# facebookresearch/generative-recommenders

Measured on NVIDIA H100. Metric: user-seqs/sec HSTU-large L=8192 d=256 bf16 fwd+bwd, higher is better.
Workload: dtype bf16

## Files before the change

### generative_recommenders_b200/_lib.py

```python
import ctypes as C
import os
from typing import Optional

import torch

_HERE = os.path.dirname(os.path.abspath(__file__))
LIB_PATH = os.environ.get("HSTU_B200_LIB") or os.path.join(_HERE, "lib", "libhstu_b200.so")

ABI_VERSION = 1
F32, BF16, F16, E4M3 = 0, 1, 2, 3
IMPL_AUTO, IMPL_GENERIC, IMPL_UMMA = 0, 1, 2

_DTYPES = {torch.float32: F32, torch.bfloat16: BF16, torch.float16: F16, torch.float8_e4m3fn: E4M3}


class AttnParams(C.Structure):
    _fields_ = [
        ("abi_version", C.c_int32), ("dtype", C.c_int32), ("impl", C.c_int32), ("batch", C.c_int32),
        ("heads", C.c_int32), ("dqk", C.c_int32), ("dv", C.c_int32), ("max_seq_len", C.c_int32),
        ("total_rows", C.c_int64), ("alpha", C.c_float), ("max_attn_len", C.c_int32),
        ("min_full_attn_seq_len", C.c_int32), ("contextual_seq_len", C.c_int32), ("delta_q_len", C.c_int32),
        ("offsets_are_i64", C.c_int32), ("num_targets_are_i64", C.c_int32),
        ("seq_offsets", C.c_void_p), ("num_targets", C.c_void_p), ("q", C.c_void_p), ("k", C.c_void_p),
        ("v", C.c_void_p), ("out", C.c_void_p),
# ... 28 lines not shown
    ]


_lib: Optional[C.CDLL] = None

_i32, _i64, _f32, _u64, _vp = C.c_int32, C.c_int64, C.c_float, C.c_uint64, C.c_void_p

_PROTOS = {
    "hstu_last_error": (C.c_char_p, []),
    "hstu_abi_version": (C.c_int, []),
    "hstu_attn_workspace_bytes": (C.c_size_t, [C.POINTER(AttnParams), C.c_int]),
    "hstu_attn_fwd": (C.c_int, [C.POINTER(AttnParams), _vp]),
    "hstu_attn_bwd": (C.c_int, [C.POINTER(AttnParams), _vp]),
    "hstu_attn_fwd_fp8": (C.c_int, [C.POINTER(AttnParams), C.POINTER(Descales), _vp]),
    "hstu_attn_select_impl": (C.c_int, [C.POINTER(AttnParams), C.c_int]),
    "hstu_mask_valid": (C.c_int, [_i32] * 7),
    "hstu_kv_range_for_q_rows": (C.c_int, [_i32] * 7 + [C.POINTER(_i32)] * 2),
    "hstu_q_range_for_kv_rows": (C.c_int, [_i32] * 7 + [C.POINTER(_i32)] * 3),
    "hstu_layer_norm_fwd": (C.c_int, [_vp, _vp, _vp, _vp, _vp, _vp, _i64, _i32, _i64, _i64, _f32, _i32, _i32, _vp]),
    "hstu_layer_norm_bwd": (C.c_int, [_vp] * 10 + [_i64, _i32, _i64, _i64, _i64, _i32, _i32, _vp]),
    "hstu_norm_bwd_partial_rows": (_i32, []),
    "hstu_rms_norm_fwd": (C.c_int, [_vp, _vp, _vp, _vp, _i64, _i32, _f32, _i32, _vp]),
    "hstu_rms_norm_bwd": (C.c_int, [_vp] * 7 + [_i64, _i32, _i32, _vp]),
    "hstu_norm_mul_dropout_fwd": (C.c_int, [_vp] * 7 + [_i64, _i32, _i32, _i64, _i64, _f32, _f32, _u64, _i32, _i32, _i32, _i32, _vp]),
    "hstu_norm_mul_dropout_bwd": (C.c_int, [_vp] * 12 + [_i64, _i32, _i32, _i64, _i64, _i64, _i64, _f32, _u64, _i32, _i32, _i32, _i32, _vp]),
    "hstu_silu_fwd": (C.c_int, [_vp, _vp, _i64, _i32, _i64, _i64, _i32, _vp]),
    "hstu_silu_bwd": (C.c_int, [_vp, _vp, _vp, _i64, _i32, _i64, _i64, _i64, _i32, _vp]),
    "hstu_jagged_concat": (C.c_int, [_vp] * 5 + [_i32] * 8 + [_vp]),
    "hstu_jagged_split": (C.c_int, [_vp] * 5 + [_i32] * 8 + [_vp]),
    "hstu_position_embeddings_fwd": (C.c_int, [_vp] * 10 + [_i64, _i32, _i32, _i32, _i32, _i32, _f32, _i32, _i32, _i32, _i32, _i32, _i32, _vp]),
# ... 117 lines not shown
```

### generative_recommenders_b200/csrc/api.cu

```cuda
#include <stdarg.h>
#include <string.h>

#include "common.cuh"
#include "internal.h"

namespace hstu {

static thread_local char g_err[512] = "";

void set_error(const char* fmt, ...) {
  va_list ap;
  va_start(ap, fmt);
  vsnprintf(g_err, sizeof(g_err), fmt, ap);
  va_end(ap);
}

static int validate_attn(const hstu_attn_params* p, bool bwd) {
  HSTU_CHECK_ARG(p != nullptr, "params is NULL");
  HSTU_CHECK_ARG(p->abi_version == HSTU_B200_ABI_VERSION, "ABI version mismatch: caller %d, library %d", p->abi_version,
                 HSTU_B200_ABI_VERSION);
  HSTU_CHECK_ARG(p->dtype == HSTU_F32 || p->dtype == HSTU_BF16 || p->dtype == HSTU_F16 || p->dtype == HSTU_E4M3, "bad dtype %d",
                 p->dtype);
  HSTU_CHECK_ARG(p->max_seq_len > 0, "max_seq_len must be larger than 0");
  HSTU_CHECK_ARG(p->batch >= 0 && p->heads > 0, "bad batch/heads");
// ... 45 lines not shown
    set_error("deterministic backward with a relative bias is not supported: the dpos_w / dts_w gradients are added "
              "with atomics");
    return HSTU_ERR_UNSUPPORTED;
  }
  const bool can = wgmma_supported(*p, bwd);
  if (p->impl == HSTU_IMPL_GENERIC) return HSTU_IMPL_GENERIC;
  if (p->impl == HSTU_IMPL_UMMA) {
    if (!can) {
      set_error("wgmma path does not support this problem (dtype=%d dqk=%d dv=%d delta=%d bias=%d)", p->dtype, p->dqk,
                p->dv, p->delta_q_len, p->pos_w != nullptr || p->ts_w != nullptr);
      return HSTU_ERR_UNSUPPORTED;
    }
    return HSTU_IMPL_UMMA;
  }
  return can ? HSTU_IMPL_UMMA : HSTU_IMPL_GENERIC;
}

static int validate_descales(const hstu_attn_descales* d) {
  if (d == nullptr) return 0;
  const float* ptr[3] = {d->q, d->k, d->v};
  const int64_t bs[3] = {d->q_batch_stride, d->k_batch_stride, d->v_batch_stride};
  const int64_t hs[3] = {d->q_head_stride, d->k_head_stride, d->v_head_stride};
  for (int i = 0; i < 3; ++i) {
    const char name = "qkv"[i];
    HSTU_CHECK_ARG(bs[i] >= 0 && hs[i] >= 0, "%c descale: negative stride (batch %lld, head %lld)", name, (long long)bs[i],
                   (long long)hs[i]);
    HSTU_CHECK_ARG((reinterpret_cast<uintptr_t>(ptr[i]) & 3) == 0, "%c descale: %p is not a float pointer", name, (const void*)ptr[i]);
  }
  return 0;
}
// ... 69 lines not shown
  if (int e = validate_attn(p, false)) return e;
  HSTU_CHECK_ARG(p->dtype == HSTU_E4M3, "hstu_attn_fwd_fp8: q, k, v must be HSTU_E4M3 (got dtype %d)", p->dtype);
  if (int e = validate_descales(descales)) return e;
  const int impl = select_impl(p, false);
  if (impl < 0) return impl;
  if (p->batch == 0 || p->total_rows == 0) return 0;
  if (int e = bind_device(p->q)) return e;
  if (int e = check_descale_devices(descales)) return e;
  if (!is_sm90()) {
    set_error("hstu_attn_fwd_fp8: the fp8 kernels need an sm_90 device");
    return HSTU_ERR_UNSUPPORTED;
  }
  hstu_attn_descales none;
  memset(&none, 0, sizeof(none));
  return attn_wgmma_fwd_e4m3(*p, descales ? *descales : none, (cudaStream_t)stream);
}

int hstu_mask_valid(int32_t len, int32_t num_targets, int32_t max_attn_len, int32_t min_full_attn_seq_len,
                    int32_t contextual_seq_len, int32_t i, int32_t j) {
  SeqMask m = make_seq_mask(len, num_targets, max_attn_len, min_full_attn_seq_len, contextual_seq_len);
  return mask_valid(m, i, j) ? 1 : 0;
}

int hstu_kv_range_for_q_rows(int32_t len, int32_t num_targets, int32_t max_attn_len, int32_t min_full_attn_seq_len,
                             int32_t contextual_seq_len, int32_t m0, int32_t m1, int32_t* lo, int32_t* hi) {
  HSTU_CHECK_ARG(lo && hi && m0 >= 0 && m1 > m0 && m1 <= len, "bad row range");
  SeqMask m = make_seq_mask(len, num_targets, max_attn_len, min_full_attn_seq_len, contextual_seq_len);
  int l, h;
  kv_range_for_q_rows(m, m0, m1, &l, &h);
  *lo = l;
// ... 202 lines not shown
```

### generative_recommenders_b200/csrc/attn_fp16_operands.cu

```cuda
#include <cuda_fp16.h>
#include <cuda_fp8.h>
#include <string.h>

#include "attn_fp16_operands.cuh"
#include "common.cuh"
#include "internal.h"

namespace hstu {

constexpr int kPreRows = 256, kPreThreads = 256, kPreD = 32;

struct PreOperand {
  const void* src;
  long long row_stride, head_stride;
  __half* dst;
};

struct PreParams {
  PreOperand op[kAmaxSlots];
  int nops;
  const void* seq_offsets;
  int offsets_i64, max_seq_len, heads;
  int d;
  float alpha;
  uint32_t* amax;
};

__device__ __forceinline__ float bf16_bits_to_float(uint32_t b) { return __uint_as_float(b << 16); }

__global__ void __launch_bounds__(kPreThreads) fp16_operands_amax_kernel(const __grid_constant__ PreParams p) {
  const int b = blockIdx.z, h = blockIdx.y;
  const long long row0 = load_index(p.seq_offsets, p.offsets_i64, b);
  const int len = min((int)(load_index(p.seq_offsets, p.offsets_i64, b + 1) - row0), p.max_seq_len);
  const int r0 = blockIdx.x * kPreRows;
  if (r0 >= len) return;
// ... 11 lines not shown
#pragma unroll
      for (int i = 0; i < 4; ++i) {
        m = max(m, (w[i] & 0x7fffu) << 16);
        m = max(m, (w[i] >> 16 & 0x7fffu) << 16);
      }
    }
#pragma unroll
    for (int s = 16; s > 0; s >>= 1) m = max(m, __shfl_xor_sync(0xffffffffu, m, s));
    if (lane == 0) red[o][warp] = m;
  }
  __syncthreads();
  if (threadIdx.x < p.nops) {
    uint32_t m = 0u;
#pragma unroll
    for (int w = 0; w < kPreThreads / 32; ++w) m = max(m, red[threadIdx.x][w]);
    if (m) atomicMax(p.amax + ((long long)b * p.heads + h) * kAmaxSlots + threadIdx.x, m);
  }
}

template <bool E4M3>
__global__ void __launch_bounds__(kPreThreads) fp16_operands_convert_kernel(const __grid_constant__ PreParams p) {
  const int b = blockIdx.z, h = blockIdx.y;
  const long long row0 = load_index(p.seq_offsets, p.offsets_i64, b);
  const int len = min((int)(load_index(p.seq_offsets, p.offsets_i64, b + 1) - row0), p.max_seq_len);
  const int r0 = blockIdx.x * kPreRows;
  if (r0 >= len) return;
  const int rows = min(kPreRows, len - r0);
  const int d = E4M3 ? p.d : kPreD, cpr = d / 8;
  int exps[kAmaxSlots] = {0, 0, 0, 0};
  if constexpr (!E4M3) {
    const OperandExps ex = operand_exps(p.amax + ((long long)b * p.heads + h) * kAmaxSlots, p.alpha, kPreD);
    exps[0] = ex.q, exps[1] = ex.k, exps[2] = ex.v, exps[3] = ex.o;
  }
  for (int o = 0; o < p.nops; ++o) {
    const PreOperand& op = p.op[o];
    const int e = exps[o];
    for (int c = threadIdx.x; c < rows * cpr; c += kPreThreads) {
      const int r = c / cpr, part = c % cpr;
      const long long row = row0 + r0 + r;
      uint32_t y[4];
      if constexpr (E4M3) {
        const uint2 x = *reinterpret_cast<const uint2*>(reinterpret_cast<const uint8_t*>(op.src) + row * op.row_stride +
                                                        (long long)h * op.head_stride + part * 8);
        const uint32_t w[2] = {x.x, x.y};
#pragma unroll
        for (int i = 0; i < 4; ++i) {
          const __half2_raw v = __nv_cvt_fp8x2_to_halfraw2((__nv_fp8x2_storage_t)(w[i >> 1] >> (16 * (i & 1))), __NV_E4M3);
          y[i] = (uint32_t)v.x | ((uint32_t)v.y << 16);
        }
      } else {
        const uint4 x = *reinterpret_cast<const uint4*>(reinterpret_cast<const uint16_t*>(op.src) + row * op.row_stride +
                                                        (long long)h * op.head_stride + part * 8);
        const uint32_t w[4] = {x.x, x.y, x.z, x.w};
#pragma unroll
        for (int i = 0; i < 4; ++i) {
          const __half2 v = __floats2half2_rn(scalbnf(bf16_bits_to_float(w[i] & 0xffffu), e), scalbnf(bf16_bits_to_float(w[i] >> 16), e));
          y[i] = *reinterpret_cast<const uint32_t*>(&v);
        }
      }
      *reinterpret_cast<uint4*>(op.dst + (row * p.heads + h) * d + part * 8) = make_uint4(y[0], y[1], y[2], y[3]);
    }
  }
}

static size_t align256(size_t n) { return (n + 255) / 256 * 256; }

size_t fp16_operands_workspace_bytes(const hstu_attn_params& p, bool bwd) {
  const size_t amax = align256((size_t)p.batch * p.heads * kAmaxSlots * sizeof(uint32_t));
  const size_t copy = align256((size_t)p.total_rows * p.heads * kPreD * sizeof(__half));
  return amax + (bwd ? 4 : 3) * copy;
}

int fp16_operands_prepass(const hstu_attn_params& p, bool bwd, Fp16Operands* out, cudaStream_t st) {
  const size_t need = fp16_operands_workspace_bytes(p, bwd);
  if (p.workspace == nullptr || p.workspace_bytes < need) {
    set_error("hstu_attn_%s: workspace of %zu bytes required (got %zu)", bwd ? "bwd" : "fwd", need, p.workspace_bytes);
    return HSTU_ERR_WORKSPACE;
  }
  uint8_t* ws = reinterpret_cast<uint8_t*>(p.workspace);
  const size_t amax_bytes = (size_t)p.batch * p.heads * kAmaxSlots * sizeof(uint32_t);
  const size_t copy = align256((size_t)p.total_rows * p.heads * kPreD * sizeof(__half));
  PreParams pp;
  memset(&pp, 0, sizeof(pp));
  pp.amax = reinterpret_cast<uint32_t*>(ws);
  const void* src[kAmaxSlots] = {p.q, p.k, p.v, p.dout};
  const long long rs[kAmaxSlots] = {p.q_row_stride, p.k_row_stride, p.v_row_stride, p.do_row_stride};
  const long long hs[kAmaxSlots] = {p.q_head_stride, p.k_head_stride, p.v_head_stride, p.do_head_stride};
  pp.nops = bwd ? 4 : 3;
  for (int o = 0; o < pp.nops; ++o) {
    pp.op[o].src = src[o];
    pp.op[o].row_stride = rs[o];
    pp.op[o].head_stride = hs[o];
    pp.op[o].dst = reinterpret_cast<__half*>(ws + align256(amax_bytes) + o * copy);
    out->copy[o] = pp.op[o].dst;
  }
  out->amax = pp.amax;
  pp.seq_offsets = p.seq_offsets;
  pp.offsets_i64 = p.offsets_are_i64;
  pp.max_seq_len = p.max_seq_len;
  pp.heads = p.heads;
  pp.alpha = p.alpha;
  HSTU_CUDA_OK(cudaMemsetAsync(pp.amax, 0, amax_bytes, st));
  if (p.batch == 0 || p.max_seq_len <= 0) return 0;
  const dim3 grid((p.max_seq_len + kPreRows - 1) / kPreRows, p.heads, p.batch);
  fp16_operands_amax_kernel<<<grid, kPreThreads, 0, st>>>(pp);
  HSTU_CUDA_OK(cudaGetLastError());
  fp16_operands_convert_kernel<false><<<grid, kPreThreads, 0, st>>>(pp);
  HSTU_CUDA_OK(cudaGetLastError());
  return 0;
}

size_t e4m3_v_copy_bytes(const hstu_attn_params& p) { return align256((size_t)p.total_rows * p.heads * p.dv * sizeof(__half)); }

int e4m3_v_prepass(const hstu_attn_params& p, const void** v16, cudaStream_t st) {
  const size_t need = e4m3_v_copy_bytes(p);
  if (p.workspace == nullptr || p.workspace_bytes < need) {
    set_error("hstu_attn_fwd_fp8: workspace of %zu bytes required (got %zu)", need, p.workspace_bytes);
    return HSTU_ERR_WORKSPACE;
  }
  PreParams pp;
  memset(&pp, 0, sizeof(pp));
  pp.nops = 1;
  pp.op[0].src = p.v;
  pp.op[0].row_stride = p.v_row_stride;
// ... 17 lines not shown
```

### generative_recommenders_b200/csrc/attn_wgmma_bwd.cu

```cuda
#include "attn_wgmma_bwd.cuh"

namespace hstu {

template <int D, bool BF16>
__global__ void __launch_bounds__(kAttnThreads, 1) attn_bwd_wgmma_kernel(const __grid_constant__ BwdParams p) {
  bwd_key_tile<D, D, BF16, true>(p);
}

template <int D, bool BF16>
__global__ void __launch_bounds__(kAttnThreads, split_min_blocks(D)) attn_bwd_dkdv_wgmma_kernel(const __grid_constant__ BwdParams p) {
  bwd_key_tile<D, D, BF16, false>(p);
}

template <int D, bool BF16>
__global__ void __launch_bounds__(kAttnThreads, split_min_blocks(D)) attn_bwd_dq_wgmma_kernel(const __grid_constant__ BwdParams p) {
  bwd_dq_body<D, D, BF16>(p);
}

template <bool BF16>
__global__ void dq_convert_kernel(const float* __restrict__ acc, uint16_t* __restrict__ dq, long long rows, int heads, int D,
                                  long long row_stride, long long head_stride, float scale) {
  const long long nvec = rows * heads * (D / 8);
  for (long long idx = (long long)blockIdx.x * blockDim.x + threadIdx.x; idx < nvec; idx += (long long)gridDim.x * blockDim.x) {
    const int v = (int)(idx % (D / 8));
// ... 88 lines not shown
      return launch_bwd_wgmma<32, false, true>(p, st, &f16);
    }
    case 64:
      if (split) return bf ? launch_bwd_wgmma<64, true, true>(p, st) : launch_bwd_wgmma<64, false, true>(p, st);
      return bf ? launch_bwd_wgmma<64, true, false>(p, st) : launch_bwd_wgmma<64, false, false>(p, st);
    case 128:
      if (split) return bf ? launch_bwd_wgmma<128, true, true>(p, st) : launch_bwd_wgmma<128, false, true>(p, st);
      return bf ? launch_bwd_wgmma<128, true, false>(p, st) : launch_bwd_wgmma<128, false, false>(p, st);
    case 256:
      return bf ? launch_bwd_wgmma<256, true, true>(p, st) : launch_bwd_wgmma<256, false, true>(p, st);
  }
  set_error("wgmma backward: unsupported head dim %d", p.dqk);
  return HSTU_ERR_UNSUPPORTED;
}

}
```

### generative_recommenders_b200/csrc/internal.h

```cpp
#pragma once
#include <cuda_runtime.h>
#include <stddef.h>

#include "../../include/hstu_b200.h"

namespace hstu {
void set_error(const char* fmt, ...);

int attn_generic_fwd(const hstu_attn_params& p, cudaStream_t st);
int attn_generic_bwd(const hstu_attn_params& p, cudaStream_t st);

bool wgmma_supported(const hstu_attn_params& p, bool bwd);
size_t wgmma_workspace_bytes(const hstu_attn_params& p, bool bwd);
int attn_wgmma_fwd(const hstu_attn_params& p, cudaStream_t st);
int attn_wgmma_bwd(const hstu_attn_params& p, cudaStream_t st);
int attn_wgmma_fwd_mixed(const hstu_attn_params& p, cudaStream_t st);
int attn_wgmma_bwd_mixed(const hstu_attn_params& p, cudaStream_t st);
bool aligned_view(const void* ptr, long long row_stride, long long head_stride);
bool wgmma_fwd_supported(const hstu_attn_params& p);
size_t wgmma_delta_workspace_bytes(const hstu_attn_params& p);

struct Fp16Operands {
  const unsigned int* amax;
  const void* copy[4];
};
size_t fp16_operands_workspace_bytes(const hstu_attn_params& p, bool bwd);
int fp16_operands_prepass(const hstu_attn_params& p, bool bwd, Fp16Operands* out, cudaStream_t st);
size_t e4m3_v_copy_bytes(const hstu_attn_params& p);
int e4m3_v_prepass(const hstu_attn_params& p, const void** v16, cudaStream_t st);

int e4m3_fwd_check(const hstu_attn_params& p);
int attn_wgmma_fwd_e4m3(const hstu_attn_params& p, const hstu_attn_descales& ds, cudaStream_t st);
int attn_wgmma_fwd_e4m3_mixed(const hstu_attn_params& p, const hstu_attn_descales& ds, const void* v16, cudaStream_t st);
bool is_sm90();

int layer_norm_fwd(const void* x, const void* w, const void* b, void* y, float* mean, float* rstd, long long n, int D,
                   long long xs, long long ys, float eps, int dtype, int swish, bool rms, cudaStream_t st);
int layer_norm_bwd(const void* dy, const void* x, const void* w, const void* b, const float* mean, const float* rstd,
                   void* dx, float* dw, float* db, float* partial, long long n, int D, long long xs, long long dys,
                   long long dxs, int dtype, int swish, bool rms, cudaStream_t st);
int norm_mul_dropout_fwd(const void* attn, const void* u, const void* w, const void* b, void* out, float* mean,
                         float* rstd, long long n, int H, int dv, long long as, long long us, float eps, float p,
// ... 46 lines not shown
```

### generative_recommenders_b200/ops/hstu_attention.py

```python
import ctypes as C
from typing import Optional, Tuple

import torch

from .. import _lib
from ..common import HammerKernel, require_cuda_kernel, switch_to_contiguous_if_needed


def _fill_common(p, max_seq_len, alpha, q, k, v, seq_offsets, num_targets, max_attn_len, contextual_seq_len,
                 min_full_attn_seq_len, impl, delta_q_len=0):
    if seq_offsets.dtype not in (torch.int32, torch.int64):
        raise RuntimeError("seq_offsets must be int32 or int64")
    if num_targets is not None and num_targets.dtype not in (torch.int32, torch.int64):
        raise RuntimeError("num_targets must be int32 or int64")
    p.abi_version = _lib.ABI_VERSION
    p.dtype = _lib.dtype_code(q)
    p.impl = impl
    p.batch = seq_offsets.numel() - 1
    p.heads = q.shape[1]
    p.dqk = q.shape[2]
    p.dv = v.shape[2]
    p.max_seq_len = int(max_seq_len)
    p.total_rows = k.shape[0]
    p.alpha = float(alpha)
# ... 14 lines not shown
def _workspace(p, bwd: bool, device):
    nbytes = _lib.lib().hstu_attn_workspace_bytes(C.byref(p), int(bwd))
    if nbytes == 0:
        p.workspace, p.workspace_bytes = None, 0
        return None
    ws = torch.empty(nbytes + 256, dtype=torch.uint8, device=device)
    base = (ws.data_ptr() + 255) // 256 * 256
    p.workspace, p.workspace_bytes = base, nbytes
    return ws


def _prep(*ts):
    return tuple(switch_to_contiguous_if_needed(t) for t in ts)


def cuda_hstu_attention_fwd(
    max_seq_len: int, alpha: float, q: torch.Tensor, k: torch.Tensor, v: torch.Tensor, seq_offsets: torch.Tensor,
    num_targets: Optional[torch.Tensor] = None, max_attn_len: int = 0, contextual_seq_len: int = 0,
    min_full_attn_seq_len: int = 0, impl: int = _lib.IMPL_AUTO, delta_q_len: int = 0,
    out: Optional[torch.Tensor] = None, bias: Optional[Tuple[torch.Tensor, torch.Tensor, torch.Tensor]] = None,
    descales: Optional[Tuple[Optional[torch.Tensor], Optional[torch.Tensor], Optional[torch.Tensor]]] = None,
) -> torch.Tensor:
    if descales is not None or any(t.dtype == _FP8 for t in (q, k, v)):
        if bias is not None or delta_q_len:
            raise RuntimeError("fp8 attention: the relative bias and delta_q are not supported")
        return cuda_hstu_attention_fwd_fp8(max_seq_len, alpha, q, k, v, seq_offsets, descales, num_targets, max_attn_len,
                                           contextual_seq_len, min_full_attn_seq_len, impl, out)
    dev = _lib.require_cuda(q, k, v, seq_offsets, num_targets)
    q, k, v = _prep(q, k, v)
    seq_offsets = seq_offsets.contiguous()
    if num_targets is not None:
        num_targets = num_targets.contiguous()
    if out is None:
        out = torch.empty((q.shape[0], q.shape[1], v.shape[2]), dtype=v.dtype, device=dev)
    p = _lib.AttnParams()
    _fill_common(p, max_seq_len, alpha, q, k, v, seq_offsets, num_targets, max_attn_len, contextual_seq_len,
                 min_full_attn_seq_len, impl, delta_q_len)
    p.out = out.data_ptr()
    p.o_row_stride, p.o_head_stride = out.stride(0), out.stride(1)
    keep = _fill_bias(p, bias, None)
    ws = _workspace(p, False, dev)
    with torch.cuda.device(dev), _lib.timed("attn_fwd", dev):
        _lib.check(_lib.lib().hstu_attn_fwd(C.byref(p), _lib.stream_ptr(dev)), "hstu_attn_fwd")
    if delta_q_len:
        _lib.note_launch(2 if ws is not None else 1)
    else:
        _lib.note_launch(3 if ws is not None else 1)
    del ws, keep
    return out


_FP8 = torch.float8_e4m3fn


def cuda_hstu_attention_fwd_fp8(
    max_seq_len: int, alpha: float, q: torch.Tensor, k: torch.Tensor, v: torch.Tensor, seq_offsets: torch.Tensor,
    descales: Optional[Tuple[Optional[torch.Tensor], Optional[torch.Tensor], Optional[torch.Tensor]]] = None,
    num_targets: Optional[torch.Tensor] = None, max_attn_len: int = 0, contextual_seq_len: int = 0,
    min_full_attn_seq_len: int = 0, impl: int = _lib.IMPL_AUTO, out: Optional[torch.Tensor] = None,
) -> torch.Tensor:
    if not all(t.dtype == _FP8 for t in (q, k, v)):
        raise RuntimeError(f"fp8 attention: q, k and v must all be torch.float8_e4m3fn (got {q.dtype}, {k.dtype}, {v.dtype}); "
# ... 29 lines not shown
    with torch.cuda.device(dev), _lib.timed("attn_fwd_fp8", dev):
        _lib.check(_lib.lib().hstu_attn_fwd_fp8(C.byref(p), C.byref(ds), _lib.stream_ptr(dev)), "hstu_attn_fwd_fp8")
    _lib.note_launch(2)
    del ws
    return out


def cuda_hstu_attention_bwd(
    max_seq_len: int, alpha: float, dout: torch.Tensor, q: torch.Tensor, k: torch.Tensor, v: torch.Tensor,
    dq: torch.Tensor, dk: torch.Tensor, dv: torch.Tensor, seq_offsets: torch.Tensor,
    num_targets: Optional[torch.Tensor] = None, max_attn_len: int = 0, contextual_seq_len: int = 0,
    min_full_attn_seq_len: int = 0, impl: int = _lib.IMPL_AUTO,
    bias: Optional[Tuple[torch.Tensor, torch.Tensor, torch.Tensor]] = None,
    dbias: Optional[Tuple[torch.Tensor, torch.Tensor]] = None,
    deterministic: Optional[bool] = None,
) -> None:
    if deterministic is None:
        deterministic = torch.are_deterministic_algorithms_enabled()
    dev = _lib.require_cuda(dout, q, k, v, dq, dk, dv, seq_offsets, num_targets)
    q, k, v, dout = _prep(q, k, v, dout)
    for g in (dq, dk, dv):
        if g.stride(-1) != 1:
            raise RuntimeError("dq/dk/dv must have a dense last dimension")
    seq_offsets = seq_offsets.contiguous()
    if num_targets is not None:
        num_targets = num_targets.contiguous()
    p = _lib.AttnParams()
    _fill_common(p, max_seq_len, alpha, q, k, v, seq_offsets, num_targets, max_attn_len, contextual_seq_len,
                 min_full_attn_seq_len, impl)
    p.dout, p.dq, p.dk, p.dv_out = dout.data_ptr(), dq.data_ptr(), dk.data_ptr(), dv.data_ptr()
    p.do_row_stride, p.do_head_stride = dout.stride(0), dout.stride(1)
    p.dq_row_stride, p.dq_head_stride = dq.stride(0), dq.stride(1)
    p.dk_row_stride, p.dk_head_stride = dk.stride(0), dk.stride(1)
    p.dv_row_stride, p.dv_head_stride = dv.stride(0), dv.stride(1)
    p.deterministic = int(bool(deterministic))
    keep = _fill_bias(p, bias, dbias)
    ws = _workspace(p, True, dev)
    with torch.cuda.device(dev), _lib.timed("attn_bwd", dev):
        _lib.check(_lib.lib().hstu_attn_bwd(C.byref(p), _lib.stream_ptr(dev)), "hstu_attn_bwd")
    _lib.note_launch(4 if ws is not None and p.dtype == _lib.BF16 and p.dqk == 32 else 2)
    del ws, keep


def _fill_bias(p, bias, dbias):
    if bias is None:
        return None
    pos_w, ts_w, timestamps = bias
    keep = []
    n, B = int(p.max_seq_len), int(p.batch)
    if pos_w is not None and pos_w.numel() != 2 * n - 1:
        raise RuntimeError(f"relative position bias: pos_w must have 2 * max_seq_len - 1 = {2 * n - 1} entries, got {pos_w.numel()}")
# ... 131 lines not shown
```

### generative_recommenders_b200/ops/hstu_compute.py

```python
from typing import Optional, Tuple

import torch

from .. import _lib
from ..common import HammerKernel, require_cuda_kernel
from .hstu_attention import cuda_hstu_attention_bwd, cuda_hstu_attention_fwd, hstu_mha
from .layer_norm import _partial, cuda_layer_norm_bwd, cuda_layer_norm_fwd, layer_norm


def cuda_silu_fwd(x: torch.Tensor) -> torch.Tensor:
    dev = _lib.require_cuda(x)
    n, c = x.shape
    y = torch.empty((n, c), dtype=x.dtype, device=dev)
    with torch.cuda.device(dev), _lib.timed("silu_fwd", dev):
        _lib.check(_lib.lib().hstu_silu_fwd(x.data_ptr(), y.data_ptr(), n, c, x.stride(0), y.stride(0), _lib.dtype_code(x),
                                            _lib.stream_ptr(dev)), "hstu_silu_fwd")
        _lib.note_launch(1)
    return y


def cuda_silu_bwd(dy: torch.Tensor, x: torch.Tensor, dx: torch.Tensor) -> None:
    dev = x.device
    n, c = x.shape
    dy = dy if dy.stride(-1) == 1 else dy.contiguous()
# ... 130 lines not shown
                                            training, concat_ux, group_norm, num_heads, linear_dim, silu_u,
                                            recompute_y_in_backward)


class _HSTUPreprocessAndAttentionFunction(torch.autograd.Function):
    @staticmethod
    def forward(ctx, x, norm_weight, norm_bias, norm_eps, num_heads, attn_dim, hidden_dim, uvqk_weight, uvqk_bias,
                max_seq_len, seq_offsets, attn_alpha, num_targets, max_attn_len, contextual_seq_len, recompute_uvqk,
                recompute_normed_x, impl):
        x = _row_major(x)
        normed_x, mean, rstd = cuda_layer_norm_fwd(x, norm_weight, norm_bias, norm_eps, False)
        uvqk = torch.addmm(uvqk_bias, normed_x, uvqk_weight)
        H, dqk, dv = num_heads, attn_dim, hidden_dim
        u_pre, v, q, k = torch.split(uvqk, [dv * H, dv * H, dqk * H, dqk * H], dim=1)
        u = cuda_silu_fwd(u_pre)
        out = cuda_hstu_attention_fwd(max_seq_len, attn_alpha, q.view(-1, H, dqk), k.view(-1, H, dqk), v.view(-1, H, dv),
                                      seq_offsets, num_targets, max_attn_len, contextual_seq_len, 0, impl)
        ctx.save_for_backward(x, norm_weight, norm_bias, uvqk_weight, uvqk_bias, mean, rstd, seq_offsets, num_targets,
                              None if recompute_normed_x else normed_x,
                              None if recompute_uvqk else uvqk)
        ctx.cfg = (norm_eps, H, dqk, dv, max_seq_len, attn_alpha, max_attn_len, contextual_seq_len, impl)
        return u, out.view(-1, H * dv)

    @staticmethod
    def backward(ctx, du, dattn):
        (x, norm_weight, norm_bias, uvqk_weight, uvqk_bias, mean, rstd, seq_offsets, num_targets, normed_x,
         uvqk) = ctx.saved_tensors
        norm_eps, H, dqk, dv, max_seq_len, alpha, max_attn_len, contextual_seq_len, impl = ctx.cfg
        if normed_x is None:
            normed_x, _, _ = cuda_layer_norm_fwd(x, norm_weight, norm_bias, norm_eps, False, save_stats=False)
        if uvqk is None:
            uvqk = torch.addmm(uvqk_bias, normed_x, uvqk_weight)
        u_pre, v, q, k = torch.split(uvqk, [dv * H, dv * H, dqk * H, dqk * H], dim=1)
        duvqk = torch.empty_like(uvqk)
        d_u, d_v, d_q, d_k = torch.split(duvqk, [dv * H, dv * H, dqk * H, dqk * H], dim=1)
        dattn = _row_major(dattn)
        cuda_hstu_attention_bwd(max_seq_len, alpha, dattn.view(-1, H, dv), q.view(-1, H, dqk), k.view(-1, H, dqk),
                                v.view(-1, H, dv), d_q.view(-1, H, dqk), d_k.view(-1, H, dqk), d_v.view(-1, H, dv),
                                seq_offsets, num_targets, max_attn_len, contextual_seq_len, 0, impl)
        cuda_silu_bwd(du, u_pre, d_u)
        d_w = torch.mm(normed_x.t(), duvqk)
        d_b = duvqk.sum(dim=0)
        d_normed = torch.mm(duvqk, uvqk_weight.t())
        dx, dnw, dnb = cuda_layer_norm_bwd(d_normed, x, norm_weight, norm_bias, mean, rstd, False)
        return (dx, dnw.to(norm_weight.dtype), dnb.to(norm_bias.dtype), None, None, None, None, d_w, d_b, None, None, None,
                None, None, None, None, None, None)


def hstu_preprocess_and_attention(
    x: torch.Tensor, norm_weight: torch.Tensor, norm_bias: torch.Tensor, norm_eps: float, num_heads: int, attn_dim: int,
    hidden_dim: int, uvqk_weight: torch.Tensor, uvqk_bias: torch.Tensor, max_seq_len: int, seq_offsets: torch.Tensor,
    attn_alpha: float, causal: bool, num_targets: Optional[torch.Tensor], max_attn_len: int, contextual_seq_len: int,
    recompute_uvqk_in_backward: bool, recompute_normed_x_in_backward: bool, sort_by_length: bool, prefill: bool = False,
    kernel: HammerKernel = HammerKernel.CUDA, impl: int = _lib.IMPL_AUTO,
# ... 22 lines not shown
```

### include/hstu_b200.h

```cpp
#ifndef HSTU_B200_H_
#define HSTU_B200_H_

#include <stddef.h>
#include <stdint.h>

#ifdef __cplusplus
extern "C" {
#endif

#define HSTU_B200_ABI_VERSION 1

typedef enum hstu_dtype { HSTU_F32 = 0, HSTU_BF16 = 1, HSTU_F16 = 2, HSTU_E4M3 = 3 } hstu_dtype;

typedef enum hstu_status {
  HSTU_OK = 0,
  HSTU_ERR_INVALID_ARGUMENT = -1,
  HSTU_ERR_UNSUPPORTED = -2,
  HSTU_ERR_CUDA = -3,
  HSTU_ERR_WORKSPACE = -4
} hstu_status;

typedef enum hstu_attn_impl {
  HSTU_IMPL_AUTO = 0,
  HSTU_IMPL_GENERIC = 1,
// ... 40 lines not shown
  const int64_t* timestamps;
  int32_t num_ts_buckets;
  int32_t deterministic;
  float* dpos_w;
  float* dts_w;
  void* workspace;
  size_t workspace_bytes;
} hstu_attn_params;

const char* hstu_last_error(void);
int hstu_abi_version(void);

size_t hstu_attn_workspace_bytes(const hstu_attn_params* p, int is_backward);
int hstu_attn_fwd(const hstu_attn_params* p, void* cuda_stream);
int hstu_attn_bwd(const hstu_attn_params* p, void* cuda_stream);

typedef struct hstu_attn_descales {
  const float* q;
  const float* k;
  const float* v;
  int64_t q_batch_stride, q_head_stride;
  int64_t k_batch_stride, k_head_stride;
  int64_t v_batch_stride, v_head_stride;
} hstu_attn_descales;
int hstu_attn_fwd_fp8(const hstu_attn_params* p, const hstu_attn_descales* descales, void* cuda_stream);
int hstu_attn_select_impl(const hstu_attn_params* p, int is_backward);

int hstu_mask_valid(int32_t len, int32_t num_targets , int32_t max_attn_len,
                    int32_t min_full_attn_seq_len, int32_t contextual_seq_len, int32_t i, int32_t j);
int hstu_kv_range_for_q_rows(int32_t len, int32_t num_targets, int32_t max_attn_len, int32_t min_full_attn_seq_len,
// ... 92 lines not shown
```

Measured before the change: 103.4.

## Keep fp16 attention operands from forward and reuse them in backward

The forward pass can now write its converted fp16 copies of q, k and v, plus their amax scales, into a buffer that is saved on the autograd context. The backward pass then converts only dout and runs the wgmma backward kernel on the kept copies. When uvqk is recomputed, only the u slice is recomputed, skipping the q/k/v part of the addmm. This removes the repeated bf16-to-fp16 prepass and part of the GEMM recompute, at the cost of holding three extra fp16 operand copies in memory between forward and backward. The path is gated to bf16 with dqk == dv == 32 on the wgmma kernels.

```diff
diff --git a/generative_recommenders_b200/_lib.py b/generative_recommenders_b200/_lib.py
--- a/generative_recommenders_b200/_lib.py
+++ b/generative_recommenders_b200/_lib.py
@@ -66,6 +66,10 @@
     "hstu_attn_bwd": (C.c_int, [C.POINTER(AttnParams), _vp]),
     "hstu_attn_fwd_fp8": (C.c_int, [C.POINTER(AttnParams), C.POINTER(Descales), _vp]),
     "hstu_attn_select_impl": (C.c_int, [C.POINTER(AttnParams), C.c_int]),
+    "hstu_attn_fp16_operands_bytes": (C.c_size_t, [C.POINTER(AttnParams)]),
+    "hstu_attn_fwd_keep_fp16_operands": (C.c_int, [C.POINTER(AttnParams), _vp, C.c_size_t, _vp]),
+    "hstu_attn_bwd_fp16_operands_workspace_bytes": (C.c_size_t, [C.POINTER(AttnParams)]),
+    "hstu_attn_bwd_on_fp16_operands": (C.c_int, [C.POINTER(AttnParams), _vp, C.c_size_t, _vp]),
     "hstu_mask_valid": (C.c_int, [_i32] * 7),
     "hstu_kv_range_for_q_rows": (C.c_int, [_i32] * 7 + [C.POINTER(_i32)] * 2),
     "hstu_q_range_for_kv_rows": (C.c_int, [_i32] * 7 + [C.POINTER(_i32)] * 3),
diff --git a/generative_recommenders_b200/csrc/api.cu b/generative_recommenders_b200/csrc/api.cu
--- a/generative_recommenders_b200/csrc/api.cu
+++ b/generative_recommenders_b200/csrc/api.cu
@@ -83,6 +83,10 @@
     return HSTU_IMPL_UMMA;
   }
   return can ? HSTU_IMPL_UMMA : HSTU_IMPL_GENERIC;
+}
+
+static bool runs_on_fp16_operands(const hstu_attn_params* p, bool bwd) {
+  return p->dtype == HSTU_BF16 && p->dqk == 32 && p->dv == 32 && p->delta_q_len == 0 && select_impl(p, bwd) == HSTU_IMPL_UMMA;
 }
 
 static int validate_descales(const hstu_attn_descales* d) {
@@ -182,6 +186,57 @@
   hstu_attn_descales none;
   memset(&none, 0, sizeof(none));
   return attn_wgmma_fwd_e4m3(*p, descales ? *descales : none, (cudaStream_t)stream);
+}
+
+size_t hstu_attn_fp16_operands_bytes(const hstu_attn_params* p) {
+  if (p == nullptr || validate_attn(p, false) != 0) return 0;
+  if (p->batch == 0 || p->total_rows == 0 || !runs_on_fp16_operands(p, false)) return 0;
+  return fp16_operands_workspace_bytes(*p, false);
+}
+
+int hstu_attn_fwd_keep_fp16_operands(const hstu_attn_params* p, void* operands, size_t operands_bytes, void* stream) {
+  if (int e = validate_attn(p, false)) return e;
+  if (p->batch == 0 || p->total_rows == 0) return 0;
+  HSTU_CHECK_ARG(operands != nullptr && (reinterpret_cast<uintptr_t>(operands) & 255) == 0,
+                 "operands must be a 256-byte aligned buffer (got %p)", operands);
+  if (int e = bind_device(p->q)) return e;
+  if (!runs_on_fp16_operands(p, false)) {
+    set_error("hstu_attn_fwd_keep_fp16_operands: only bf16 at dqk == dv == 32 on the wgmma kernels runs on fp16 operands");
+    return HSTU_ERR_UNSUPPORTED;
+  }
+  const size_t need = fp16_operands_workspace_bytes(*p, false);
+  HSTU_CHECK_ARG(operands_bytes >= need, "operands buffer of %zu bytes required (got %zu)", need, operands_bytes);
+  hstu_attn_params c = *p;
+  c.workspace = operands;
+  c.workspace_bytes = need;
+  return attn_wgmma_fwd(c, (cudaStream_t)stream);
+}
+
+size_t hstu_attn_bwd_fp16_operands_workspace_bytes(const hstu_attn_params* p) {
+  if (p == nullptr || p->batch <= 0 || p->heads <= 0 || p->total_rows <= 0) return 0;
+  return fp16_operands_dout_workspace_bytes(*p);
+}
+
+int hstu_attn_bwd_on_fp16_operands(const hstu_attn_params* p, const void* operands, size_t operands_bytes, void* stream) {
+  HSTU_CHECK_ARG(p != nullptr, "params is NULL");
+  HSTU_CHECK_ARG(operands != nullptr && (reinterpret_cast<uintptr_t>(operands) & 255) == 0,
+                 "operands must be a 256-byte aligned buffer (got %p)", operands);
+  hstu_attn_params c = *p;
+  const Fp16Operands kept = fp16_operands_at(c, const_cast<void*>(operands));
+  c.q = kept.copy[0], c.k = kept.copy[1], c.v = kept.copy[2];
+  c.q_row_stride = c.k_row_stride = c.v_row_stride = (int64_t)c.heads * c.dqk;
+  c.q_head_stride = c.k_head_stride = c.v_head_stride = c.dqk;
+  if (int e = validate_attn(&c, true)) return e;
+  if (c.batch == 0 || c.total_rows == 0) return 0;
+  const size_t need = fp16_operands_workspace_bytes(c, false);
+  HSTU_CHECK_ARG(operands_bytes >= need, "operands buffer of %zu bytes required (got %zu): not kept by a forward of these sizes",
+                 need, operands_bytes);
+  if (int e = bind_device(c.dout)) return e;
+  if (!runs_on_fp16_operands(&c, true)) {
+    set_error("hstu_attn_bwd_on_fp16_operands: only bf16 at dqk == dv == 32 on the wgmma kernels runs on fp16 operands");
+    return HSTU_ERR_UNSUPPORTED;
+  }
+  return attn_wgmma_bwd_on_fp16_operands(c, operands, (cudaStream_t)stream);
 }
 
 int hstu_mask_valid(int32_t len, int32_t num_targets, int32_t max_attn_len, int32_t min_full_attn_seq_len,
diff --git a/generative_recommenders_b200/csrc/attn_fp16_operands.cu b/generative_recommenders_b200/csrc/attn_fp16_operands.cu
--- a/generative_recommenders_b200/csrc/attn_fp16_operands.cu
+++ b/generative_recommenders_b200/csrc/attn_fp16_operands.cu
@@ -19,6 +19,7 @@
 struct PreParams {
   PreOperand op[kAmaxSlots];
   int nops;
+  int slot0;
   const void* seq_offsets;
   int offsets_i64, max_seq_len, heads;
   int d;
@@ -60,7 +61,7 @@
     uint32_t m = 0u;
 #pragma unroll
     for (int w = 0; w < kPreThreads / 32; ++w) m = max(m, red[threadIdx.x][w]);
-    if (m) atomicMax(p.amax + ((long long)b * p.heads + h) * kAmaxSlots + threadIdx.x, m);
+    if (m) atomicMax(p.amax + ((long long)b * p.heads + h) * kAmaxSlots + p.slot0 + threadIdx.x, m);
   }
 }
 
@@ -80,7 +81,7 @@
   }
   for (int o = 0; o < p.nops; ++o) {
     const PreOperand& op = p.op[o];
-    const int e = exps[o];
+    const int e = exps[p.slot0 + o];
     for (int c = threadIdx.x; c < rows * cpr; c += kPreThreads) {
       const int r = c / cpr, part = c % cpr;
       const long long row = row0 + r0 + r;
@@ -110,11 +111,36 @@
 }
 
 static size_t align256(size_t n) { return (n + 255) / 256 * 256; }
+static size_t amax_bytes(const hstu_attn_params& p) { return (size_t)p.batch * p.heads * kAmaxSlots * sizeof(uint32_t); }
+static size_t copy_bytes(const hstu_attn_params& p) { return align256((size_t)p.total_rows * p.heads * kPreD * sizeof(__half)); }
 
 size_t fp16_operands_workspace_bytes(const hstu_attn_params& p, bool bwd) {
-  const size_t amax = align256((size_t)p.batch * p.heads * kAmaxSlots * sizeof(uint32_t));
-  const size_t copy = align256((size_t)p.total_rows * p.heads * kPreD * sizeof(__half));
-  return amax + (bwd ? 4 : 3) * copy;
+  return align256(amax_bytes(p)) + (bwd ? 4 : 3) * copy_bytes(p);
+}
+
+size_t fp16_operands_dout_workspace_bytes(const hstu_attn_params& p) { return align256(amax_bytes(p)) + copy_bytes(p); }
+
+Fp16Operands fp16_operands_at(const hstu_attn_params& p, void* buf) {
+  uint8_t* base = reinterpret_cast<uint8_t*>(buf);
+  Fp16Operands f;
+  f.amax = reinterpret_cast<uint32_t*>(base);
+  for (int o = 0; o < kAmaxSlots; ++o) f.copy[o] = base + align256(amax_bytes(p)) + o * copy_bytes(p);
+  return f;
+}
+
+static int launch_prepass(const hstu_attn_params& p, PreParams& pp, cudaStream_t st) {
+  pp.seq_offsets = p.seq_offsets;
+  pp.offsets_i64 = p.offsets_are_i64;
+  pp.max_seq_len = p.max_seq_len;
+  pp.heads = p.heads;
+  pp.alpha = p.alpha;
+  if (p.batch == 0 || p.max_seq_len <= 0) return 0;
+  const dim3 grid((p.max_seq_len + kPreRows - 1) / kPreRows, p.heads, p.batch);
+  fp16_operands_amax_kernel<<<grid, kPreThreads, 0, st>>>(pp);
+  HSTU_CUDA_OK(cudaGetLastError());
+  fp16_operands_convert_kernel<false><<<grid, kPreThreads, 0, st>>>(pp);
+  HSTU_CUDA_OK(cudaGetLastError());
+  return 0;
 }
 
 int fp16_operands_prepass(const hstu_attn_params& p, bool bwd, Fp16Operands* out, cudaStream_t st) {
@@ -123,12 +149,10 @@
     set_error("hstu_attn_%s: workspace of %zu bytes required (got %zu)", bwd ? "bwd" : "fwd", need, p.workspace_bytes);
     return HSTU_ERR_WORKSPACE;
   }
-  uint8_t* ws = reinterpret_cast<uint8_t*>(p.workspace);
-  const size_t amax_bytes = (size_t)p.batch * p.heads * kAmaxSlots * sizeof(uint32_t);
-  const size_t copy = align256((size_t)p.total_rows * p.heads * kPreD * sizeof(__half));
+  *out = fp16_operands_at(p, p.workspace);
   PreParams pp;
   memset(&pp, 0, sizeof(pp));
-  pp.amax = reinterpret_cast<uint32_t*>(ws);
+  pp.amax = const_cast<uint32_t*>(out->amax);
   const void* src[kAmaxSlots] = {p.q, p.k, p.v, p.dout};
   const long long rs[kAmaxSlots] = {p.q_row_stride, p.k_row_stride, p.v_row_stride, p.do_row_stride};
   const long long hs[kAmaxSlots] = {p.q_head_stride, p.k_head_stride, p.v_head_stride, p.do_head_stride};
@@ -137,23 +161,33 @@
     pp.op[o].src = src[o];
     pp.op[o].row_stride = rs[o];
     pp.op[o].head_stride = hs[o];
-    pp.op[o].dst = reinterpret_cast<__half*>(ws + align256(amax_bytes) + o * copy);
-    out->copy[o] = pp.op[o].dst;
-  }
-  out->amax = pp.amax;
-  pp.seq_offsets = p.seq_offsets;
-  pp.offsets_i64 = p.offsets_are_i64;
-  pp.max_seq_len = p.max_seq_len;
-  pp.heads = p.heads;
-  pp.alpha = p.alpha;
-  HSTU_CUDA_OK(cudaMemsetAsync(pp.amax, 0, amax_bytes, st));
-  if (p.batch == 0 || p.max_seq_len <= 0) return 0;
-  const dim3 grid((p.max_seq_len + kPreRows - 1) / kPreRows, p.heads, p.batch);
-  fp16_operands_amax_kernel<<<grid, kPreThreads, 0, st>>>(pp);
-  HSTU_CUDA_OK(cudaGetLastError());
-  fp16_operands_convert_kernel<false><<<grid, kPreThreads, 0, st>>>(pp);
-  HSTU_CUDA_OK(cudaGetLastError());
-  return 0;
+    pp.op[o].dst = reinterpret_cast<__half*>(const_cast<void*>(out->copy[o]));
+  }
+  HSTU_CUDA_OK(cudaMemsetAsync(pp.amax, 0, amax_bytes(p), st));
+  return launch_prepass(p, pp, st);
+}
+
+int fp16_operands_dout_prepass(const hstu_attn_params& p, const void* kept, Fp16Operands* out, cudaStream_t st) {
+  const size_t need = fp16_operands_dout_workspace_bytes(p);
+  if (p.workspace == nullptr || p.workspace_bytes < need) {
+    set_error("hstu_attn_bwd_on_fp16_operands: workspace of %zu bytes required (got %zu)", need, p.workspace_bytes);
+    return HSTU_ERR_WORKSPACE;
+  }
+  const Fp16Operands k = fp16_operands_at(p, const_cast<void*>(kept)), w = fp16_operands_at(p, p.workspace);
+  out->amax = w.amax;
+  for (int o = 0; o < 3; ++o) out->copy[o] = k.copy[o];
+  out->copy[kAmaxDO] = w.copy[0];
+  PreParams pp;
+  memset(&pp, 0, sizeof(pp));
+  pp.amax = const_cast<uint32_t*>(w.amax);
+  pp.nops = 1;
+  pp.slot0 = kAmaxDO;
+  pp.op[0].src = p.dout;
+  pp.op[0].row_stride = p.do_row_stride;
+  pp.op[0].head_stride = p.do_head_stride;
+  pp.op[0].dst = reinterpret_cast<__half*>(const_cast<void*>(w.copy[0]));
+  HSTU_CUDA_OK(cudaMemcpyAsync(pp.amax, k.amax, amax_bytes(p), cudaMemcpyDeviceToDevice, st));
+  return launch_prepass(p, pp, st);
 }
 
 size_t e4m3_v_copy_bytes(const hstu_attn_params& p) { return align256((size_t)p.total_rows * p.heads * p.dv * sizeof(__half)); }
diff --git a/generative_recommenders_b200/csrc/attn_wgmma_bwd.cu b/generative_recommenders_b200/csrc/attn_wgmma_bwd.cu
--- a/generative_recommenders_b200/csrc/attn_wgmma_bwd.cu
+++ b/generative_recommenders_b200/csrc/attn_wgmma_bwd.cu
@@ -126,4 +126,10 @@
   return HSTU_ERR_UNSUPPORTED;
 }
 
+int attn_wgmma_bwd_on_fp16_operands(const hstu_attn_params& p, const void* kept, cudaStream_t st) {
+  Fp16Operands f16;
+  if (int e = fp16_operands_dout_prepass(p, kept, &f16, st)) return e;
+  return launch_bwd_wgmma<32, false, true>(p, st, &f16);
 }
+
+}
diff --git a/generative_recommenders_b200/csrc/internal.h b/generative_recommenders_b200/csrc/internal.h
--- a/generative_recommenders_b200/csrc/internal.h
+++ b/generative_recommenders_b200/csrc/internal.h
@@ -14,6 +14,7 @@
 size_t wgmma_workspace_bytes(const hstu_attn_params& p, bool bwd);
 int attn_wgmma_fwd(const hstu_attn_params& p, cudaStream_t st);
 int attn_wgmma_bwd(const hstu_attn_params& p, cudaStream_t st);
+int attn_wgmma_bwd_on_fp16_operands(const hstu_attn_params& p, const void* kept, cudaStream_t st);
 int attn_wgmma_fwd_mixed(const hstu_attn_params& p, cudaStream_t st);
 int attn_wgmma_bwd_mixed(const hstu_attn_params& p, cudaStream_t st);
 bool aligned_view(const void* ptr, long long row_stride, long long head_stride);
@@ -25,7 +26,10 @@
   const void* copy[4];
 };
 size_t fp16_operands_workspace_bytes(const hstu_attn_params& p, bool bwd);
+Fp16Operands fp16_operands_at(const hstu_attn_params& p, void* buf);
 int fp16_operands_prepass(const hstu_attn_params& p, bool bwd, Fp16Operands* out, cudaStream_t st);
+size_t fp16_operands_dout_workspace_bytes(const hstu_attn_params& p);
+int fp16_operands_dout_prepass(const hstu_attn_params& p, const void* kept, Fp16Operands* out, cudaStream_t st);
 size_t e4m3_v_copy_bytes(const hstu_attn_params& p);
 int e4m3_v_prepass(const hstu_attn_params& p, const void** v16, cudaStream_t st);
 
diff --git a/generative_recommenders_b200/ops/hstu_attention.py b/generative_recommenders_b200/ops/hstu_attention.py
--- a/generative_recommenders_b200/ops/hstu_attention.py
+++ b/generative_recommenders_b200/ops/hstu_attention.py
@@ -52,12 +52,26 @@
     return tuple(switch_to_contiguous_if_needed(t) for t in ts)
 
 
+def _wgmma_view(t: torch.Tensor) -> torch.Tensor:
+    ok = t.data_ptr() % 16 == 0 and t.stride(0) % 8 == 0 and t.stride(1) % 8 == 0
+    return t if ok else t.clone(memory_format=torch.contiguous_format)
+
+
+class Fp16Operands:
+
+    def __init__(self):
+        self.buf: Optional[torch.Tensor] = None
+        self.base = 0
+        self.nbytes = 0
+
+
 def cuda_hstu_attention_fwd(
     max_seq_len: int, alpha: float, q: torch.Tensor, k: torch.Tensor, v: torch.Tensor, seq_offsets: torch.Tensor,
     num_targets: Optional[torch.Tensor] = None, max_attn_len: int = 0, contextual_seq_len: int = 0,
     min_full_attn_seq_len: int = 0, impl: int = _lib.IMPL_AUTO, delta_q_len: int = 0,
     out: Optional[torch.Tensor] = None, bias: Optional[Tuple[torch.Tensor, torch.Tensor, torch.Tensor]] = None,
     descales: Optional[Tuple[Optional[torch.Tensor], Optional[torch.Tensor], Optional[torch.Tensor]]] = None,
+    fp16_operands: Optional[Fp16Operands] = None,
 ) -> torch.Tensor:
     if descales is not None or any(t.dtype == _FP8 for t in (q, k, v)):
         if bias is not None or delta_q_len:
@@ -77,13 +91,23 @@
     p.out = out.data_ptr()
     p.o_row_stride, p.o_head_stride = out.stride(0), out.stride(1)
     keep = _fill_bias(p, bias, None)
-    ws = _workspace(p, False, dev)
-    with torch.cuda.device(dev), _lib.timed("attn_fwd", dev):
-        _lib.check(_lib.lib().hstu_attn_fwd(C.byref(p), _lib.stream_ptr(dev)), "hstu_attn_fwd")
+    kept = _lib.lib().hstu_attn_fp16_operands_bytes(C.byref(p)) if fp16_operands is not None else 0
+    if kept:
+        fp16_operands.buf = torch.empty(kept + 256, dtype=torch.uint8, device=dev)
+        fp16_operands.base = (fp16_operands.buf.data_ptr() + 255) // 256 * 256
+        fp16_operands.nbytes = kept
+        ws = None
+        with torch.cuda.device(dev), _lib.timed("attn_fwd", dev):
+            _lib.check(_lib.lib().hstu_attn_fwd_keep_fp16_operands(C.byref(p), fp16_operands.base, kept, _lib.stream_ptr(dev)),
+                       "hstu_attn_fwd_keep_fp16_operands")
+    else:
+        ws = _workspace(p, False, dev)
+        with torch.cuda.device(dev), _lib.timed("attn_fwd", dev):
+            _lib.check(_lib.lib().hstu_attn_fwd(C.byref(p), _lib.stream_ptr(dev)), "hstu_attn_fwd")
     if delta_q_len:
         _lib.note_launch(2 if ws is not None else 1)
     else:
-        _lib.note_launch(3 if ws is not None else 1)
+        _lib.note_launch(3 if ws is not None or kept else 1)
     del ws, keep
     return out
 
@@ -143,14 +167,22 @@
     bias: Optional[Tuple[torch.Tensor, torch.Tensor, torch.Tensor]] = None,
     dbias: Optional[Tuple[torch.Tensor, torch.Tensor]] = None,
     deterministic: Optional[bool] = None,
+    fp16_operands: Optional[Fp16Operands] = None,
 ) -> None:
     if deterministic is None:
         deterministic = torch.are_deterministic_algorithms_enabled()
+    kept = fp16_operands is not None and fp16_operands.buf is not None
+    if kept and q is None:
+        q = k = v = dout
     dev = _lib.require_cuda(dout, q, k, v, dq, dk, dv, seq_offsets, num_targets)
     q, k, v, dout = _prep(q, k, v, dout)
     for g in (dq, dk, dv):
         if g.stride(-1) != 1:
             raise RuntimeError("dq/dk/dv must have a dense last dimension")
+    grads = (dq, dk, dv)
+    if kept:
+        dout = _wgmma_view(dout)
+        dq, dk, dv = (_wgmma_view(g) for g in grads)
     seq_offsets = seq_offsets.contiguous()
     if num_targets is not None:
         num_targets = num_targets.contiguous()
@@ -164,6 +196,20 @@
     p.dv_row_stride, p.dv_head_stride = dv.stride(0), dv.stride(1)
     p.deterministic = int(bool(deterministic))
     keep = _fill_bias(p, bias, dbias)
+    if kept:
+        p.q = p.k = p.v = None
+        nbytes = _lib.lib().hstu_attn_bwd_fp16_operands_workspace_bytes(C.byref(p))
+        ws = torch.empty(nbytes + 256, dtype=torch.uint8, device=dev)
+        p.workspace, p.workspace_bytes = (ws.data_ptr() + 255) // 256 * 256, nbytes
+        with torch.cuda.device(dev), _lib.timed("attn_bwd", dev):
+            _lib.check(_lib.lib().hstu_attn_bwd_on_fp16_operands(C.byref(p), fp16_operands.base, fp16_operands.nbytes,
+                                                                 _lib.stream_ptr(dev)), "hstu_attn_bwd_on_fp16_operands")
+        _lib.note_launch(4)
+        for g, w in zip(grads, (dq, dk, dv)):
+            if w is not g:
+                g.copy_(w)
+        del ws, keep
+        return
     ws = _workspace(p, True, dev)
     with torch.cuda.device(dev), _lib.timed("attn_bwd", dev):
         _lib.check(_lib.lib().hstu_attn_bwd(C.byref(p), _lib.stream_ptr(dev)), "hstu_attn_bwd")
diff --git a/generative_recommenders_b200/ops/hstu_compute.py b/generative_recommenders_b200/ops/hstu_compute.py
--- a/generative_recommenders_b200/ops/hstu_compute.py
+++ b/generative_recommenders_b200/ops/hstu_compute.py
@@ -4,7 +4,7 @@
 
 from .. import _lib
 from ..common import HammerKernel, require_cuda_kernel
-from .hstu_attention import cuda_hstu_attention_bwd, cuda_hstu_attention_fwd, hstu_mha
+from .hstu_attention import Fp16Operands, cuda_hstu_attention_bwd, cuda_hstu_attention_fwd, hstu_mha
 from .layer_norm import _partial, cuda_layer_norm_bwd, cuda_layer_norm_fwd, layer_norm
 
 
@@ -168,8 +168,10 @@
         H, dqk, dv = num_heads, attn_dim, hidden_dim
         u_pre, v, q, k = torch.split(uvqk, [dv * H, dv * H, dqk * H, dqk * H], dim=1)
         u = cuda_silu_fwd(u_pre)
+        ops = Fp16Operands()
         out = cuda_hstu_attention_fwd(max_seq_len, attn_alpha, q.view(-1, H, dqk), k.view(-1, H, dqk), v.view(-1, H, dv),
-                                      seq_offsets, num_targets, max_attn_len, contextual_seq_len, 0, impl)
+                                      seq_offsets, num_targets, max_attn_len, contextual_seq_len, 0, impl, fp16_operands=ops)
+        ctx.fp16_operands = ops
         ctx.save_for_backward(x, norm_weight, norm_bias, uvqk_weight, uvqk_bias, mean, rstd, seq_offsets, num_targets,
                               None if recompute_normed_x else normed_x,
                               None if recompute_uvqk else uvqk)
@@ -181,17 +183,23 @@
         (x, norm_weight, norm_bias, uvqk_weight, uvqk_bias, mean, rstd, seq_offsets, num_targets, normed_x,
          uvqk) = ctx.saved_tensors
         norm_eps, H, dqk, dv, max_seq_len, alpha, max_attn_len, contextual_seq_len, impl = ctx.cfg
+        ops = ctx.fp16_operands
         if normed_x is None:
             normed_x, _, _ = cuda_layer_norm_fwd(x, norm_weight, norm_bias, norm_eps, False, save_stats=False)
-        if uvqk is None:
-            uvqk = torch.addmm(uvqk_bias, normed_x, uvqk_weight)
-        u_pre, v, q, k = torch.split(uvqk, [dv * H, dv * H, dqk * H, dqk * H], dim=1)
-        duvqk = torch.empty_like(uvqk)
+        if uvqk is None and ops.buf is not None:
+            u_pre = torch.addmm(uvqk_bias[:dv * H], normed_x, uvqk_weight[:, :dv * H])
+            q = k = v = None
+        else:
+            if uvqk is None:
+                uvqk = torch.addmm(uvqk_bias, normed_x, uvqk_weight)
+            u_pre, v, q, k = torch.split(uvqk, [dv * H, dv * H, dqk * H, dqk * H], dim=1)
+            q, k, v = q.view(-1, H, dqk), k.view(-1, H, dqk), v.view(-1, H, dv)
+        duvqk = torch.empty((normed_x.shape[0], uvqk_weight.shape[1]), dtype=normed_x.dtype, device=normed_x.device)
         d_u, d_v, d_q, d_k = torch.split(duvqk, [dv * H, dv * H, dqk * H, dqk * H], dim=1)
         dattn = _row_major(dattn)
-        cuda_hstu_attention_bwd(max_seq_len, alpha, dattn.view(-1, H, dv), q.view(-1, H, dqk), k.view(-1, H, dqk),
-                                v.view(-1, H, dv), d_q.view(-1, H, dqk), d_k.view(-1, H, dqk), d_v.view(-1, H, dv),
-                                seq_offsets, num_targets, max_attn_len, contextual_seq_len, 0, impl)
+        cuda_hstu_attention_bwd(max_seq_len, alpha, dattn.view(-1, H, dv), q, k, v, d_q.view(-1, H, dqk), d_k.view(-1, H, dqk),
+                                d_v.view(-1, H, dv), seq_offsets, num_targets, max_attn_len, contextual_seq_len, 0, impl,
+                                fp16_operands=ops)
         cuda_silu_bwd(du, u_pre, d_u)
         d_w = torch.mm(normed_x.t(), duvqk)
         d_b = duvqk.sum(dim=0)
diff --git a/include/hstu_b200.h b/include/hstu_b200.h
--- a/include/hstu_b200.h
+++ b/include/hstu_b200.h
@@ -78,6 +78,12 @@
 size_t hstu_attn_workspace_bytes(const hstu_attn_params* p, int is_backward);
 int hstu_attn_fwd(const hstu_attn_params* p, void* cuda_stream);
 int hstu_attn_bwd(const hstu_attn_params* p, void* cuda_stream);
+
+size_t hstu_attn_fp16_operands_bytes(const hstu_attn_params* p);
+int hstu_attn_fwd_keep_fp16_operands(const hstu_attn_params* p, void* operands, size_t operands_bytes, void* cuda_stream);
+size_t hstu_attn_bwd_fp16_operands_workspace_bytes(const hstu_attn_params* p);
+int hstu_attn_bwd_on_fp16_operands(const hstu_attn_params* p, const void* operands, size_t operands_bytes,
+                                   void* cuda_stream);
 
 typedef struct hstu_attn_descales {
   const float* q;
```

Measured after the change: 106.8, median of 6. 3.3% higher.
